# baowj-678/koordinator

Measured on AMD Instinct MI355X. Metric: pods placed/sec + (pod,node) Filter+Score evals/sec at 50k nodes, 1-8 GPUs, higher is better.
Workload: dtype int64; 1 GPU; config4: 50000 nodes x 100000 pods, 30% BE, NodeResourcesFit + LoadAwareScheduling, shipped scheduler-config.yaml profile; nodes=50000, pods=100000, batch_pods=24, pipeline_lag=2, parallelism=node-shard x1

## Files before the change

### koordinator_amd/csrc/api.hip

```cpp
#include <hip/hip_runtime.h>
#include <rccl/rccl.h>

#include <algorithm>
#include <array>
#include <cmath>
#include <condition_variable>
#include <memory>
#include <mutex>
#include <cstdio>
#include <cstdlib>
#include <cstring>
#include <chrono>
#include <string>
#include <unordered_map>
#include <vector>

#include "../../include/koordhip.h"
#include "cls.h"
#include "diag.h"
#include "diag_ext.h"
#include "reasons.h"
#include "preempt.h"
#include "kernels.h"
#include "place_plan.hpp"
// ... 2028 lines not shown
  int e = place_staged_impl(c);
  c->diag_valid = !e;
  if (e && c->group) c->group->abort();
  if (!e && std::getenv("KOORDHIP_PMC_REPLAY") && std::getenv("KOORDHIP_SERIAL")) e = pmc_replay(c);
  return e;
}

}

namespace {

kh::PlaceKnobs read_place_knobs() {
  const auto on = [](const char *name) { return std::getenv(name) != nullptr; };
  const auto num = [](const char *name, int32_t unset) {
    const char *v = std::getenv(name);
    return v ? std::atoi(v) : unset;
  };
  kh::PlaceKnobs k;
  k.SERIAL = on("KOORDHIP_SERIAL"), k.ROUND_LAUNCH = on("KOORDHIP_ROUND_LAUNCH");
  k.ONE_EVAL_STREAM = on("KOORDHIP_ONE_EVAL_STREAM"), k.CLS_OFF = on("KOORDHIP_CLS_OFF");
  k.SHARD_LOCAL_SIM = on("KOORDHIP_SHARD_LOCAL_SIM"), k.SHARD_FORCE = on("KOORDHIP_SHARD_FORCE");
  k.LAG1 = on("KOORDHIP_LAG1"), k.LAG2 = on("KOORDHIP_LAG2"), k.EXT_SEQ = on("KOORDHIP_EXT_SEQ");
  k.CHAIN_OFF = on("KOORDHIP_CHAIN_OFF"), k.STAMPS = on("KOORDHIP_STAMPS");
  k.NO_PRELOAD = on("KOORDHIP_NO_PRELOAD"), k.NO_KEY_TABLES = on("KOORDHIP_NO_KEY_TABLES");
  k.EXT_LEAD = num("KOORDHIP_EXT_LEAD", k.EXT_LEAD);
  k.CHAIN_PASSES = num("KOORDHIP_CHAIN_PASSES", k.CHAIN_PASSES);
  k.TRACE_POD = num("KOORDHIP_TRACE_POD", k.TRACE_POD);
  return k;
}

kh::PlaceFacts place_facts(const koordhip_ctx *c) {
  kh::PlaceFacts f;
  f.n = c->n, f.batch = c->batch, f.n_staged = c->n_staged, f.world = c->world, f.n_cu = c->n_cu;
  f.nbins = c->nbins, f.monotone = c->monotone;
  f.n_classes = (int32_t)c->cls_rep.size(), f.n_ext = (int32_t)c->ext_idx.size();
  f.has_comm = c->comm != nullptr, f.has_comm2 = c->comm2 != nullptr, f.has_group = c->group != nullptr;
  f.side = c->side, f.resv = c->resv, f.side_mode = kh::side_mode(c->dc);
  f.seq_profile = c->seq_profile, f.seq_ext_only = c->seq_ext_only, f.seq_snap = c->seq_snap;
  f.staged_ext = c->staged_ext, f.staged_ext_dev = c->staged_ext_dev, f.podx_staged = c->podx_staged;
  f.staged_reserve = c->staged_reserve, f.resv_dev_slot = c->d.dv.rslot != nullptr;
  f.resolve_lds_bytes = kh::resolve_lds_bytes;
  f.cls_run_lds = kh::cls_run_lds;
  return f;
}

int ensure_devout(koordhip_ctx *c) {
// ... 367 lines not shown
  HIP_TRY(hipMemsetAsync(pc->sync, 0, kh::kPipeSyncBytes, c->stream));
  HIP_TRY(hipEventRecord(c->ev_start, c->stream));
  HIP_TRY(hipStreamWaitEvent(c->rstream, c->ev_start, 0));
  if (plan.two) HIP_TRY(hipStreamWaitEvent(c->stream2, c->ev_start, 0));
  if (plan.rounds <= 0) return 0;
  if (plan.cls) {
    if (int e = cls_plan(c, plan.P, plan.lag, plan.K)) return e;
    if (int e = cls_alloc(c, c->n)) return e;
    if (int e = cls_reset(c)) return e;
    HIP_TRY(hipEventRecord(c->ev_start, c->stream));
    HIP_TRY(hipStreamWaitEvent(c->stream2, c->ev_start, 0));
    return 0;
  }
  for (int slot = 0; slot < (plan.two ? 2 : 1); slot++) {
    hipStream_t es = slot ? c->stream2 : c->stream;
    if (int e = eval_buffers(c, std::min(plan.P, c->n_staged), pc->lo, pc->hi, slot, es, plan.K)) return e;
    if (c->eval_fused) HIP_TRY(hipMemsetAsync(c->d_etk_sync[slot], 0, 2 * kh::kSelMaxPods * sizeof(uint32_t), es));
  }
  return 0;
}

int launch_resolve_rounds(koordhip_ctx *c, const PlaceCall &pc, int32_t r0, int32_t r1, int32_t mono, int32_t lag,
                          hipStream_t s) {
  HIP_TRY(kh::launch_resolve(c->dc, c->d, c->d_desc, c->d_pods, c->n_staged, pc.plan.P, pc.plan.K, r0, r1,
                             pc.plan.exch ? c->d_final : c->d_lists, (int64_t)kListBuf, mono, lag, pc.sync, c->d_mod,
                             c->d_out, c->d_cpus, c->d_dbg, pc.knobs.TRACE_POD, pc.knobs.NO_PRELOAD,
                             pc.knobs.NO_KEY_TABLES, s));
  c->resolve_kernel = kh::last_resolve_kernel();
  return 0;
}

int enqueue_resolve(koordhip_ctx *c, PlaceCall *pc) {
  if (!pc->plan.persistent || pc->plan.rounds <= 0) return 0;
  if (int e = timed_begin(c, TK_RESOLVE, c->rstream, &pc->res_tm)) return e;
  return launch_resolve_rounds(c, *pc, 0, pc->plan.rounds, pc->plan.mono, pc->plan.lag, c->rstream);
}

int enqueue_class_lists(koordhip_ctx *c, const PlaceCall &pc) {
  const kh::PlacePlan &plan = pc.plan;
  if (!plan.cls || plan.rounds <= 0) return 0;
  hipStream_t cs = c->stream;
  int32_t tm = -1;
  if (int e = timed_begin(c, TK_SCAN, cs, &tm)) return e;
  HIP_TRY(kh::launch_cls_run(c->dc, c->d, c->d_cls_pod, (int32_t)c->cls_rep.size(), c->d_plan + c->plan_off[0],
                             c->d_plan + c->plan_off[1], c->d_plan + c->plan_off[2], c->d_pod_cls, c->d_out, plan.lag,
                             plan.P, c->n_staged, c->d_cls_buf, c->d_cls_meta, plan.K, c->monotone, c->d_lists,
                             (int64_t)kListBuf, cls_sync(c, pc.sync), c->d_dbg ? c->d_dbg + 64 : nullptr, cs));
// ... 148 lines not shown
  if (plan.cls) {
    uint64_t q[32];
    HIP_TRY(hipMemcpy(q, c->d_dbg + 64, sizeof(q), hipMemcpyDeviceToHost));
    const double nl = (double)std::max<uint64_t>(q[7], 1), nc = (double)std::max<uint64_t>(q[15], 1);
    std::fprintf(stderr, "[koordhip stamps] class lists, cycles per launch (workgroup 0, %llu launches): buffer %.0f  log %.0f  "
                 "touched keys %.0f  compaction %.0f  sort %.0f  merge %.0f  outputs %.0f | builds (%llu): histogram %.0f  "
                 "fine %.0f  emit %.0f  sort %.0f  write %.0f\n", (unsigned long long)q[7], q[0] / nl, q[1] / nl, q[2] / nl,
                 q[3] / nl, q[4] / nl, q[5] / nl, q[6] / nl, (unsigned long long)q[15], q[8] / nc, q[9] / nc, q[10] / nc,
                 q[11] / nc, q[12] / nc);
  }
  {
    uint64_t q[4] = {0, 0, 0, 0}, rw[8] = {0, 0, 0, 0, 0, 0, 0, 0};
    HIP_TRY(hipMemcpy(q, c->d_dbg + 90, sizeof(q), hipMemcpyDeviceToHost));
    HIP_TRY(hipMemcpy(rw, c->d_dbg + 107, sizeof(rw), hipMemcpyDeviceToHost));
    std::fprintf(stderr, "[koordhip stamps] chain re-walks: walk + keys %llu (entries + claims %llu, row + evaluation "
                 "%llu)  winners' rows %llu cycles | winner rows loaded from HBM %llu\n", (unsigned long long)rw[0],
                 (unsigned long long)rw[5], (unsigned long long)rw[6], (unsigned long long)rw[1],
                 (unsigned long long)rw[2]);
    std::fprintf(stderr, "[koordhip stamps] chained decisions: %llu cycles, %llu pods resolved | claim tables %llu  "
                 "re-walks %llu  re-check + closure %llu  final table %llu | rounds with a lazy "
                 "claim table %llu\n", (unsigned long long)h[62],
                 (unsigned long long)h[63], (unsigned long long)q[0], (unsigned long long)q[1],
                 (unsigned long long)q[2], (unsigned long long)q[3], (unsigned long long)rw[7]);
  }
  if (plan.ext_pipe) {
    uint64_t q[8];
    HIP_TRY(hipMemcpy(q, c->d_dbg + 80, sizeof(q), hipMemcpyDeviceToHost));
    const double np = (double)std::max<uint64_t>(q[6], 1);
    std::fprintf(stderr, "[koordhip stamps] device pods (k_ext_pre / k_ext_final): %llu, resolve cycles from the "
                 "hand-off to the answer %llu (%.0f per pod) | final launch per pod: workgroup 0 evaluate + fold "
                 "%.0f | last workgroup: decide + publish %.0f  device commit %.0f\n",
                 (unsigned long long)h[31], (unsigned long long)h[30], h[31] ? (double)h[30] / h[31] : 0.0,
                 q[0] / np, q[3] / np, q[4] / np);
    uint64_t r[16];
    HIP_TRY(hipMemcpy(r, c->d_dbg + 96, sizeof(r), hipMemcpyDeviceToHost));
    std::fprintf(stderr, "[koordhip stamps] device-pod finals: workgroups with a full (device) re-evaluation %llu, "
                 "their re-evaluation %.2f us each\n", (unsigned long long)r[14], r[14] ? r[15] * 0.01 / r[14] : 0.0);
    const double nb = (double)std::max<uint64_t>(r[10], 1);
    std::fprintf(stderr, "[koordhip stamps] device-pod finals, us: request seen -> last workgroup arrived %.2f per pod | "
                 "per workgroup: -> gate seen %.2f  X marked %.2f  re-evaluated %.2f  folded + arrived %.2f\n",
                 r[5] * 0.01 / np, r[6] * 0.01 / nb, r[7] * 0.01 / nb, r[8] * 0.01 / nb, r[9] * 0.01 / nb);
    std::fprintf(stderr, "[koordhip stamps] device-pod hand-offs, us per pod: the request seen -> published %.2f | "
                 "requests already set when the final's first workgroup started: %llu of %llu | pre-evaluation "
                 "published after the request: %llu pods, waited %.2f us each\n",
                 r[2] * 0.01 / np, (unsigned long long)r[0], (unsigned long long)q[6], (unsigned long long)r[1],
                 r[1] ? r[3] * 0.01 / r[1] : 0.0);
// ... 979 lines not shown
```

### koordinator_amd/csrc/kernels.h

```cpp
#pragma once
#include <hip/hip_runtime.h>

#include "eval.hpp"
#include "place_plan.hpp"

namespace kh {

struct PrepIn {
  const int64_t *used_m[2];
  const int64_t *total_m[2];
  const int64_t *prod_used_m[2];
  const int64_t *thr[2];
  const int64_t *prod_thr[2];
  const uint8_t *la_flags;
};

hipError_t launch_prep_flags(const PrepIn &in, const DevNodes &d, const int32_t *rows, int32_t m, hipStream_t s);
hipError_t launch_eval_full(const DevCfg &c, const DevNodes &d, const DevPod *pods, int32_t n_pods,
                            uint8_t *status, int32_t *scores, hipStream_t s);
int32_t scan_chunks(int R, int32_t lo, int32_t hi);
hipError_t launch_scan(int R, const DevCfg &c, const DevNodes &d, const DevPod *pods, int32_t n_pods, int32_t lo,
                       int32_t hi, uint16_t *S, int64_t s_stride, uint16_t *Mx, int32_t m_stride, hipStream_t s);
struct PipeSync;
constexpr int kSelGMax = 16;
constexpr int kSelMaxPods = 64;
constexpr size_t kSelPartKeys = (size_t)kSelMaxPods * kSelGMax * 128;
int32_t select_split_groups(int32_t m, int32_t G);
hipError_t launch_select_split(const uint16_t *S, int64_t s_stride, int32_t lo, int32_t m, int32_t n_pods, int32_t k,
                               int32_t nbins, const uint16_t *Mx, int32_t m_stride, int32_t nchunks, int32_t G,
                               uint64_t *part, uint32_t *cnt, uint64_t *out, PipeSync *sync, int32_t sel_par,
                               hipStream_t s);
int32_t eval_topk_slices(int VT, int32_t lo, int32_t hi);
int eval_topk_vt(int nm, int32_t n_cu, int32_t n_pods, int32_t lo, int32_t hi, int32_t k, int knob);
hipError_t launch_eval_topk(const DevCfg &c, const DevNodes &d, const DevPod *pods, int32_t n_pods, int32_t lo,
                            int32_t hi, int32_t k, int VT, uint64_t *part, int32_t *pcnt, uint32_t *arrive,
                            uint64_t *out, PipeSync *sync, int32_t sel_par, int G, uint64_t *dbg, hipStream_t s);
hipError_t launch_topk_merge(const uint64_t *in, int64_t pod_stride, int64_t list_stride, int32_t n_pods, int32_t L,
                             int32_t k, int32_t score_bits, uint64_t *out, PipeSync *sync, int32_t sel_par,
                             hipStream_t s);
template <typename T>
hipError_t launch_scatter(T *dst, const T *src, const int32_t *idx, int32_t m, hipStream_t s);
hipError_t launch_scatter_rows(void *dst, const void *src, const int32_t *idx, int32_t m, int32_t bytes, hipStream_t s);
int side_mode(const DevCfg &c);
const char *last_eval_kernel();
const char *last_resolve_kernel();

int32_t resolve_lds_bytes(int32_t n_pods_max, int32_t k, int32_t n_nodes, int nm, int32_t lag);
hipError_t launch_resolve(const DevCfg &c, const DevNodes &d, const DevNodes *d_desc, const DevPod *pods, int32_t total, int32_t P, int32_t k,
                          int32_t r_begin, int32_t r_end, const uint64_t *lists0, int64_t list_buf, int32_t monotone,
                          int32_t lag, PipeSync *sync, int32_t *mbuf, int32_t *out_node, uint64_t *out_cpus, uint64_t *dbg,
                          int32_t trace, bool no_preload, bool no_key_tables, hipStream_t s);
hipError_t launch_wait_resolved(PipeSync *sync, int32_t rounds, hipStream_t s);
constexpr size_t kPipeSyncBytes = 384 + 4 * (1 + 128);
constexpr int kPipeSyncErrWord = 3;
constexpr int kPipeSyncExtReqWord = 32, kPipeSyncExtDoneWord = 64;
hipError_t launch_commit(const DevCfg &c, const DevNodes &d, const DevPod *pod, int32_t node, int32_t sign,
                         uint64_t *cpus, int32_t *rc, hipStream_t s);

}
```

### koordinator_amd/csrc/kernels.hip

```cpp
#include <hip/hip_runtime.h>

#include <algorithm>
#include <cstdio>

#include "eval.hpp"
#include "karg.hpp"
#include "kernels.h"
#include "pipe.hpp"
#include "rows.hpp"

namespace kh {


__device__ __forceinline__ uint64_t shfl_u64(uint64_t v, int src) {
  uint32_t lo = __shfl((uint32_t)v, src, 64);
  uint32_t hi = __shfl((uint32_t)(v >> 32), src, 64);
  return ((uint64_t)hi << 32) | lo;
}
__device__ __forceinline__ uint64_t shfl_up_u64(uint64_t v, int d) {
  uint32_t lo = __shfl_up((uint32_t)v, d, 64);
  uint32_t hi = __shfl_up((uint32_t)(v >> 32), d, 64);
  return ((uint64_t)hi << 32) | lo;
}
__device__ __forceinline__ uint64_t shfl_xor_u64(uint64_t v, int m) {
// ... 1135 lines not shown
static_assert(sizeof(NV) == RES_WORDS * 8, "NV row = 20 words");
static_assert(offsetof(NV, r) == 40 && offsetof(NV, nz_cpu) == 80 && offsetof(NV, la_u_cpu) == 112 &&
                  offsetof(NV, la_up_cpu) == 128 && offsetof(NV, a_pods) == 144 && offsetof(NV, npods) == 148 &&
                  offsetof(NV, flags) == 152,
              "NV word layout");

__device__ __forceinline__ NV slot_row(const NV &src) {
  NV v = src;
  uint32_t f = v.flags & ~(uint32_t)(NF_OVER_CPU | NF_OVER_MEM | NF_OVER_EPH);
  if (v.r[KOORDHIP_RES_CPU] > v.a[KOORDHIP_RES_CPU]) f |= NF_OVER_CPU;
  if (v.r[KOORDHIP_RES_MEM] > v.a[KOORDHIP_RES_MEM]) f |= NF_OVER_MEM;
  if (v.r[KOORDHIP_RES_EPH] > v.a[KOORDHIP_RES_EPH]) f |= NF_OVER_EPH;
  v.flags = f;
  return v;
}

struct ResLds {
  int32_t dep;
  int32_t lists, pods, prev_rows, prev_numa, cur_rows, cur_numa, hash_node, hash_slot, pre_rows, pre_numa, pre_node,
      dec_key, dec_n, dec_src, dec_e, dec_c, moved, mhash, gbits, kpre, ktab, ready, classes, modmap, total;
  int32_t kwide;
  int32_t overlap, lists2, pods2, pre_rows2, pre_numa2, pre_node2;
  int32_t ptab;
};

__host__ __device__ inline int32_t res_align(int32_t x) { return (x + 15) & ~15; }

__host__ __device__ inline int32_t res_ptab_bytes(int32_t nrow) {
  if (nrow == 0) return res_align((int32_t)offsetof(DevNodes, nu));
  return nrow == (int32_t)sizeof(NumaRow) ? res_align((int32_t)offsetof(DevNodes, rv)) : 0;
}

__host__ __device__ inline ResLds res_lds(int32_t n_pods_max, int32_t kp, int32_t n_nodes, int32_t nrow,
                                          bool overlap = false, bool tables = true, int32_t lag = 1,
                                          bool wide = false, bool chain = true) {
  const bool numa = nrow > 0;
  ResLds o;
  int32_t at = 0;
  const int32_t bitmap = res_align(((n_nodes + 31) >> 5) * 4);
  o.lists = at;
  at += res_align(n_pods_max * kp * 8);
  o.pods = at;
  at += res_align(n_pods_max * (int32_t)sizeof(DevPod));
  const int32_t rows_b = res_align(lag * n_pods_max * (int32_t)sizeof(NV));
  const int32_t numa_b = numa ? res_align(lag * n_pods_max * nrow) : 0;
  o.prev_rows = at;
// ... 4 lines not shown
  at += rows_b + numa_b;
  o.hash_node = at;
  at += RES_HASH * 4;
  o.hash_slot = at;
  at += RES_HASH * 4;
  o.pre_rows = at;
  at += res_align(RES_PRE * (int32_t)sizeof(NV));
  o.pre_numa = at;
  at += numa ? res_align(RES_PRE * nrow) : 0;
  o.pre_node = at;
  at += RES_PRE * 4;
  o.dec_key = at;
  at += RES_MAXP_ROUND * 8;
  o.dec_n = at;
  at += RES_MAXP_ROUND * 4;
  o.dec_src = at;
  at += RES_MAXP_ROUND * 4;
  o.dec_e = at;
  at += RES_MAXP_ROUND * RES_WE * 4;
  o.dec_c = at;
  at += RES_MAXP_ROUND * 4;
  o.dep = chain ? at : -1;
  at += chain ? RES_MAXP_ROUND * 8 : 0;
  o.moved = at;
  at += RES_MAXP_ROUND * 4;
  o.mhash = at;
  at += 2 * RES_MAXP_ROUND * 4;
  o.gbits = at;
  at += bitmap;
  o.kpre = o.ktab = -1;
  o.kwide = wide ? 1 : 0;
  o.ready = at;
  at += RES_MAXP_ROUND * 4;
  if (tables) {
    o.kpre = at;
    at += RES_MAXP_ROUND * RES_MAXP_ROUND * (wide ? 4 : 2);
    o.ktab = at;
    at += RES_MAXP_ROUND * RES_MAXP_ROUND * (wide ? 4 : 2);
  }
  o.classes = at;
  at += numa ? NUMA_LDS_CLASSES * (int32_t)sizeof(DevNumaClass) : 0;
  o.modmap = at;
  at += bitmap;
  o.ptab = res_ptab_bytes(nrow) ? at : -1;
  at += res_ptab_bytes(nrow);
  o.overlap = overlap ? 1 : 0;
  o.lists2 = o.pods2 = o.pre_rows2 = o.pre_numa2 = o.pre_node2 = 0;
  if (overlap) {
    o.lists2 = at;
    at += res_align(n_pods_max * kp * 8);
    o.pods2 = at;
    at += res_align(n_pods_max * (int32_t)sizeof(DevPod));
    o.pre_rows2 = at;
    at += res_align(RES_PRE * (int32_t)sizeof(NV));
    o.pre_numa2 = at;
    at += numa ? res_align(RES_PRE * nrow) : 0;
    o.pre_node2 = at;
    at += RES_PRE * 4;
  }
  o.total = at;
  return o;
}

__device__ __forceinline__ uint32_t res_hash(int32_t node) { return ((uint32_t)node * 2654435761u) >> 24; }
__device__ __forceinline__ DevPod uniform_pod(const DevPod &src) {
  DevPod p;
  const uint32_t *s = reinterpret_cast<const uint32_t *>(&src);
  uint32_t *o = reinterpret_cast<uint32_t *>(&p);
#pragma unroll
  for (int i = 0; i < (int)(sizeof(DevPod) / 4); i++) o[i] = __builtin_amdgcn_readfirstlane(s[i]);
  return p;
}
__device__ __forceinline__ bool xbit(const uint32_t *m, int32_t nd) { return (m[nd >> 5] >> (nd & 31)) & 1u; }
__device__ __forceinline__ uint64_t ktab_key(uint32_t v, int32_t nd) {
  return v ? ((uint64_t)v << 32) | (uint64_t)(0xFFFFFFFFu - (uint32_t)nd) : 0ull;
}

__global__ void k_wait_resolved(PipeSync *sy, int32_t rounds) {
  if (threadIdx.x == 0) (void)wait_at_least(&sy->res_round, rounds, sy);
}

template <int NM, bool DBG>
__global__ __launch_bounds__(res_threads<NM>()) void k_resolve(DevCfg c, const DevNodes *__restrict__ dn, int32_t n_nodes,
                                                                 const DevNumaClass *__restrict__ ncls, const DevPod *__restrict__ pods,
                                                                 int32_t total, int32_t P, int32_t k, int32_t kp,
                                                                 int32_t r_begin, int32_t r_end,
                                                                 int32_t *__restrict__ mbuf,
                                                                 const uint64_t *__restrict__ lists0,
                                                                 int64_t list_buf, int32_t monotone, int32_t lag,
                                                                 PipeSync *sy, ResLds ofs, int32_t *__restrict__ out_node,
                                                                 uint64_t *__restrict__ out_cpus,
                                                                 uint64_t *__restrict__ dbg, int32_t trace) {
  constexpr int RES_THREADS = res_threads<NM>();
  constexpr bool NUMA = NM != 0, ZONES = NM == 2;
  if constexpr (!DBG) dbg = nullptr;
  using NR = side_row_t<NM>;
  (void)trace;
  extern __shared__ __attribute__((aligned(16))) char lds[];
  uint64_t *lk = reinterpret_cast<uint64_t *>(lds + ofs.lists);
  DevPod *lpod = reinterpret_cast<DevPod *>(lds + ofs.pods);
  NV *prow = reinterpret_cast<NV *>(lds + ofs.prev_rows);
  NR *pnr = reinterpret_cast<NR *>(lds + ofs.prev_numa);
  NV *mrow = reinterpret_cast<NV *>(lds + ofs.cur_rows);
  NR *mnr = reinterpret_cast<NR *>(lds + ofs.cur_numa);
  int32_t *hnode = reinterpret_cast<int32_t *>(lds + ofs.hash_node);
  int32_t *hslot = reinterpret_cast<int32_t *>(lds + ofs.hash_slot);
  NV *pre = reinterpret_cast<NV *>(lds + ofs.pre_rows);
// ... 32 lines not shown
  __shared__ int32_t seg_w[RES_MAXP_ROUND];
  __shared__ int32_t ckey[RES_HASH], cval[RES_HASH];
  __shared__ int32_t sh_mp, sh_stop, sh_done, sh_chain;
  __shared__ uint64_t sh_rsv;
  const int t = threadIdx.x, lane = lane_id();
  const int32_t words = (n_nodes + 31) >> 5;
  const int32_t HP = max(1, RES_PRE / P);
  auto nodes = [&]() -> decltype(auto) {
    if constexpr (NM <= 2) {
      return *reinterpret_cast<const DevNodes *>(lds + ofs.ptab);
    } else {
      const DevNodes *p = dn;
      asm volatile("" : "+s"(p));
      return DevNodes(*p);
    }
  };
  if constexpr (NM <= 2) {
    constexpr int PW = (int)((NUMA ? offsetof(DevNodes, rv) : offsetof(DevNodes, nu)) / 8);
    static_assert(PW <= RES_THREADS, "one 8-byte word of the pointer table per thread");
    if (t < PW) reinterpret_cast<uint64_t *>(lds + ofs.ptab)[t] = reinterpret_cast<const uint64_t *>(dn)[t];
  }
  const bool two = kp > 64;
  const bool chain_on = (monotone & 2) && ofs.dep >= 0;
  const uint64_t t_kernel = (dbg && t == 0) ? stamp() : 0;
  if (t == 0) {
    sh_mp = r_begin > 0 ? min(mbuf[0], P) : 0;
    sh_stop = 0;
  }
  for (int32_t x = t; x < words; x += RES_THREADS) {
    modmap[x] = 0;
    gbits[x] = 0;
  }
  for (int32_t x = t; x < RES_MAXP_ROUND; x += RES_THREADS) {
    moved[x] = 0;
    ready[x] = 0;
  }
  for (int32_t x = t; x < RES_HASH; x += RES_THREADS) {
    ckey[x] = -1;
    cval[x] = 64;
  }
  const DevNumaClass *cls = ncls;
  if constexpr (NUMA) {
    const int32_t nc = dn->nu.ncls;
    if (nc <= NUMA_LDS_CLASSES) {
      uint4 *dst = reinterpret_cast<uint4 *>(lds + ofs.classes);
      const uint4 *src = reinterpret_cast<const uint4 *>(ncls);
// ... 20 lines not shown
  auto word_doff = [](int q) -> int32_t {
    if (q >= 5 && q < 10) return (q - 5) * 8;
    if (q == 10 || q == 11) return (int32_t)offsetof(DevPod, nz_cpu_m) + (q - 10) * 8;
    if (q == 14 || q == 16) return (int32_t)offsetof(DevPod, est_cpu);
    if (q == 15 || q == 17) return (int32_t)offsetof(DevPod, est_mem);
    return -1;
  };
  const int32_t doff = word_doff(lane);
  uint64_t c_pro = 0, c_wait = 0, c_loop = 0, c_rel = 0, c_hash = 0, c_wb = 0;
  uint64_t c_w1wait = 0, c_w1load = 0, c_bar = 0;
  uint64_t c_l[4] = {0, 0, 0, 0};
  uint64_t n_slow = 0, n_miss = 0, n_staged = 0, n_bulk = 0, n_tab = 0;
  uint64_t c_g[2] = {0, 0};
  uint64_t c_nx[8] = {0, 0, 0, 0, 0, 0, 0, 0};
  uint64_t c_p[3] = {0, 0, 0}, n_p2 = 0, n_conf = 0, n_slowc = 0, n_void = 0;
  uint64_t c_cand = 0, n_evpass = 0, n_tready = 0;
  uint64_t c_gc[3] = {0, 0, 0}, n_ghit = 0;
  uint64_t c_chain = 0;
  uint64_t c_ch[4] = {0, 0, 0, 0};
  uint64_t c_rw[4] = {0, 0, 0, 0}, n_chbm = 0;
  uint64_t n_lazy = 0;
  uint64_t c_ext = 0, n_ext = 0;
  auto load_round = [&](int32_t rr, int32_t rp0, int32_t rn, uint64_t *Lk, DevPod *Lp, NV *Pr, NR *Pn,
                        int32_t *Pnode, int32_t tid, int32_t nth) {
    const uint64_t *L = lists0 + (size_t)(rr & (2 * lag - 1)) * list_buf;
    const int32_t tot = rn * k;
    uint64_t he[2] = {0, 0};
    bool hv[2];
#pragma unroll
    for (int u = 0; u < 2; u++) {
      const int32_t sl = tid + u * nth, j = sl / HP, q = sl - j * HP;
      hv[u] = sl < RES_PRE && j < rn && q < k;
      if (u * nth < RES_PRE) he[u] = L[min(j * k + q, tot - 1)];
    }
    constexpr int LB = 6;
    const uint4 *L4 = reinterpret_cast<const uint4 *>(L);
    const int32_t n16 = (tot + 1) >> 1;
    auto put = [&](int32_t e, uint64_t v) {
      if (e < tot) {
        const int32_t j = e / k, q = e - j * k;
        Lk[j * kp + q] = v;
      }
    };
    auto put2 = [&](int32_t x, const uint4 &w) {
      if (x < n16) {
        put(2 * x, ((uint64_t)w.y << 32) | w.x);
        put(2 * x + 1, ((uint64_t)w.w << 32) | w.z);
      }
    };
// ... 63 lines not shown
        }
      }
      Pnode[sl] = nd[u];
    }
    for (int32_t sl = tid + 2 * nth; sl < RES_PRE; sl += nth) {
      const int32_t j = sl / HP, q = sl - j * HP;
      int32_t n1 = -1;
      if (j < rn && q < k) {
        const uint64_t e = L[(size_t)j * k + q];
        if (e != 0) n1 = key_node(e);
      }
      if (n1 >= 0) {
        NV v1;
        load_row(v1, nodes(), n1);
        Pr[sl] = v1;
        if constexpr (NUMA) {
          NR rr2;
          load_side_row<NM>(rr2, nodes(), n1);
          Pn[sl] = rr2;
        }
      }
      Pnode[sl] = n1;
    }
  };
  auto prev_slot = [&](int32_t nd) -> int32_t {
    uint32_t h = res_hash(nd);
    for (;;) {
      const int32_t x = hnode[h];
      if (x == nd) return hslot[h];
      if (x < 0) return -1;
      h = (h + 1) & (RES_HASH - 1);
    }
  };
  for (int32_t r = r_begin, p0 = r_begin * P; r < r_end && p0 < total; r++, p0 += P) {
    const int32_t n_pods = min(P, total - p0);
    const bool preloaded = ofs.overlap && r > r_begin;
    const uint64_t t_w0 = (dbg && t == 0) ? stamp() : 0;
    if (!preloaded) {
      if (t == 0 && !wait_at_least(&sy->sel[r & 1], P * (r >> 1) + n_pods, sy)) sh_stop = 1;
      __syncthreads();
    }
    if (sh_stop) return;
    const uint64_t t_entry = (dbg && t == 0) ? stamp() : 0;
    const int32_t mp = sh_mp;
    if (!preloaded) load_round(r, p0, n_pods, lk, lpod, pre, prenr, pre_node, t, RES_THREADS);
    for (int32_t x = t; x < RES_HASH; x += RES_THREADS) hnode[x] = -1;
    if (t == 0) {
      sh_done = 0;
      sh_chain = 0;
    }
    __syncthreads();
    if (t < mp) {
      const int32_t nd = pnode[t];
      uint32_t h = res_hash(nd);
      while (atomicCAS(&hnode[h], -1, nd) != -1) h = (h + 1) & (RES_HASH - 1);
      hslot[h] = t;
    }
    __syncthreads();
    const uint64_t t_a = (dbg && t == 0) ? stamp() : 0;
    if (mp > 0 && t < RES_PRE) {
      const int32_t nd = pre_node[t];
      if (nd >= 0 && prev_slot(nd) >= 0) pre_node[t] = -1;
    }
    for (int32_t base = 0; base < n_pods * RES_WE; base += RES_THREADS) {
      const int32_t x = base + t;
      const int32_t l = x / RES_WE, q = x - l * RES_WE;
      const bool live = l < n_pods;
      const uint64_t e = (live && q < kp) ? lk[l * kp + q] : 0ull;
      const int32_t nd = e ? key_node(e) : -1;
      const bool inx = e != 0 && xbit(modmap, nd);
      const int g = lane & ~(RES_WE - 1);
      const uint32_t bx = (uint32_t)(__ballot(live && e != 0 && !inx) >> g) & 0xFFu;
      const uint32_t bz = (uint32_t)(__ballot(live && e == 0) >> g) & 0xFFu;
      const int f = bx ? __builtin_ctz(bx) : RES_WE, z = bz ? __builtin_ctz(bz) : RES_WE;
      const bool general = f == RES_WE && z == RES_WE;
      const bool walked = live && !general && (q < min(f, z) || (q == f && f < z));
      uint64_t key = 0;
      int32_t ms = -1;
      if (walked) {
        if (q < min(f, z)) {
          ms = prev_slot(nd);
          const DevPod pod = lpod[l];
          key = make_key(eval_row<NM>(pod, slot_row(prow[ms]), pnr[ms], cls, c), nd);
        } else {
          key = e;
        }
      }
      uint64_t mx = key;
#pragma unroll
      for (int m = 1; m < RES_WE; m <<= 1) {
        const uint64_t o = shfl_xor_u64(mx, m);
        mx = o > mx ? o : mx;
      }
      if (live) {
        dec_e[l * RES_WE + q] = walked ? nd : -1;
        if (walked && key == mx && mx != 0) {
          int32_t src;
          if (ms >= 0) {
            src = -ms - 1;
          } else if (q < HP && pre_node[l * HP + q] == nd) {
            src = l * HP + q;
          } else {
            src = l * HP;
            if (dbg) n_p2++;
            NV v;
            load_row(v, nodes(), nd);
            pre[src] = v;
            if constexpr (NUMA) {
              NR nr;
              load_side_row<NM>(nr, nodes(), nd);
              prenr[src] = nr;
            }
            pre_node[src] = nd;
          }
          dec_src[l] = src;
        }
        if (q == 0) {
          const int32_t dn = general ? -1 : (f < z ? f + 1 : z);
          dec_key[l] = mx;
          dec_n[l] = dn;
          if (mx == 0 || dn < 0) dec_src[l] = 0;
          const uint32_t fl = lpod[l].flags;
          bool slow = !monotone || dn < 0;
          if constexpr (NM == 0) slow = slow || (fl & KH_POD_EXT) != 0u;
          if constexpr (NUMA) {
            slow = slow || (numa_on(c) && ((fl & KOORDHIP_POD_CPUSET) || c.zones) &&
                            !(fl & (KOORDHIP_POD_NUMA_SKIP | KOORDHIP_POD_NUMA_ERROR)));
          }
          if constexpr (NM >= 3) {
            slow = slow || lpod[l].resv_match != 0ull;
          }
          dec_c[l] = slow ? 2 : 0;
          if (!slow && mx != 0) {
            const int32_t sw = key_node(mx);
            uint32_t h = res_hash(sw);
            for (;;) {
              const int32_t prev = atomicCAS(&ckey[h], -1, sw);
              if (prev == -1 || prev == sw) {
                atomicMin(&cval[h], l);
                break;
              }
              h = (h + 1) & (RES_HASH - 1);
            }
          }
        }
      }
    }
    const uint64_t t_p1 = (dbg && t == 0) ? stamp() : 0;
    __syncthreads();
    const uint64_t t_p2 = (dbg && t == 0) ? stamp() : 0;
    for (int32_t x = t; x < n_pods * RES_WE; x += RES_THREADS) {
      const int32_t l = x / RES_WE;
      const int32_t y = dec_e[x];
      if (y >= 0 && !(dec_c[l] & 2)) {
        uint32_t h = res_hash(y);
        for (;;) {
          const int32_t xk = ckey[h];
          if (xk == y) {
            if (cval[h] < l) atomicOr(&dec_c[l], 1);
            break;
          }
          if (xk < 0) break;
          h = (h + 1) & (RES_HASH - 1);
        }
      }
    }
    __syncthreads();
    uint64_t *dep = ofs.dep >= 0 ? reinterpret_cast<uint64_t *>(lds + ofs.dep) : nullptr;
    if (dep)
      for (int32_t x = t; x < n_pods; x += RES_THREADS) dep[x] = 0ull;
    if (dbg && t == 0) {
      const uint64_t t_p3 = stamp();
      c_hash += t_a - t_entry;
      c_pro += t_p3 - t_a;
      c_wait += t_entry - t_w0;
      c_p[0] += t_p1 - t_a;
      c_p[1] += t_p2 - t_p1;
      c_p[2] += t_p3 - t_p2;
    }
    if (t < 64) {
      __builtin_amdgcn_s_setprio(3);
      auto wsync = [&]() {
        asm volatile("s_waitcnt lgkmcnt(0)" ::: "memory");
        __builtin_amdgcn_fence(__ATOMIC_SEQ_CST, "wavefront");
      };
      bool claims_stale = false;
      auto claims = [&]() {
        for (int32_t x = lane; x < RES_HASH; x += 64) {
          ckey[x] = -1;
          cval[x] = 64;
        }
        wsync();
        if (lane < n_pods && dec_c[lane] == 0 && dec_key[lane] != 0ull) {
          const int32_t sw2 = key_node(dec_key[lane]);
          uint32_t h = res_hash(sw2);
          for (;;) {
            const int32_t prev = atomicCAS(&ckey[h], -1, sw2);
            if (prev == -1 || prev == sw2) {
              atomicMin(&cval[h], lane);
              break;
            }
            h = (h + 1) & (RES_HASH - 1);
          }
        }
        wsync();
      };
      if (chain_on) {
        const uint64_t t_c0 = dbg ? stamp() : 0;
        auto claimer_of = [&](int32_t y) -> int32_t {
          uint32_t q = res_hash(y);
          for (;;) {
            const int32_t xk = ckey[q];
            if (xk == y) return cval[q];
            if (xk == -1) return 64;
            q = (q + 1) & (RES_HASH - 1);
          }
        };
        auto drop_conflicting = [&]() {
          if (lane < n_pods && dec_c[lane] == 1 && dec_key[lane] != 0ull) {
            const int32_t y = key_node(dec_key[lane]);
            uint32_t q = res_hash(y);
            for (;;) {
              const int32_t xk = ckey[q];
              if (xk == y) {
                if (cval[q] == lane) ckey[q] = -2;
                break;
              }
              if (xk == -1) break;
              q = (q + 1) & (RES_HASH - 1);
            }
          }
// ... 622 lines not shown
        pgen[sidx] = r - 1;
      }
      moved[lane] = 0;
      const uint64_t t_rel = dbg ? stamp() : 0;
      if (dbg) c_wb += t_rel - t_wb;
      if (lane == 0) {
        sh_mp = nm + ns;
        asm volatile("s_waitcnt vmcnt(0)" ::: "memory");
        __hip_atomic_store(&sy->res_round, r + 1, __ATOMIC_RELAXED, __HIP_MEMORY_SCOPE_AGENT);
      }
      if (dbg) {
        const uint64_t t_end = stamp();
        c_rel += t_end - t_rel;
        c_loop += t_end - t_loop;
      }
    } else if (t < 64 * (1 + res_loaders<NM>())) {
      if (ofs.overlap && r + 1 < r_end && p0 + P < total) {
        const int32_t np2 = min(P, total - (p0 + P));
        int ok = 1;
        const uint64_t t1 = dbg ? stamp() : 0;
        if (lane == 0) ok = wait_at_least(&sy->sel[(r + 1) & 1], P * ((r + 1) >> 1) + np2, sy) ? 1 : 0;
        const uint64_t t2 = dbg ? stamp() : 0;
        if (__builtin_amdgcn_readfirstlane(ok)) {
          load_round(r + 1, p0 + P, np2, lk2, lpod2, pre2, prenr2, pre_node2, t - 64, 64 * res_loaders<NM>());
          if (dbg) {
            asm volatile("s_waitcnt vmcnt(0) lgkmcnt(0)" ::: "memory");
            c_w1load += stamp() - t2;
          }
        } else if (lane == 0) {
          sh_stop = 1;
        }
        if (dbg) c_w1wait += t2 - t1;
      }
    } else {
      const int hw = __builtin_amdgcn_readfirstlane((t >> 6) - 1 - res_loaders<NM>()),
                nh = RES_THREADS / 64 - 1 - res_loaders<NM>();
      if (chain_on)
        while (!__hip_atomic_load(&sh_chain, __ATOMIC_ACQUIRE, __HIP_MEMORY_SCOPE_WORKGROUP)) __builtin_amdgcn_s_sleep(1);
      uint64_t todo = __ballot(lane < n_pods && dec_c[lane] == 1);
      for (int32_t x = 0; x < hw && todo; x++) todo &= todo - 1ull;
      for (; have_tables && todo;) {
        const int32_t l = (int32_t)__builtin_ctzll(todo);
        for (int32_t x = 0; x < nh && todo; x++) todo &= todo - 1ull;
        if (__hip_atomic_load(&sh_done, __ATOMIC_RELAXED, __HIP_MEMORY_SCOPE_WORKGROUP)) break;
        const DevPod pod = uniform_pod(lpod[l]);
        for (int32_t b0 = 0; b0 < l + mp; b0 += 64) {
          const int32_t x = b0 + lane;
// ... 21 lines not shown
        if (lane == 0) __hip_atomic_store(&ready[l], 1, __ATOMIC_RELEASE, __HIP_MEMORY_SCOPE_WORKGROUP);
      }
    }
    const uint64_t t_bar = (dbg && t == 0) ? stamp() : 0;
    __syncthreads();
    if (dbg && t == 0) c_bar += stamp() - t_bar;
    for (int32_t x = t; x < RES_MAXP_ROUND; x += RES_THREADS) ready[x] = 0;
    if (ofs.overlap) {
      uint64_t *a = lk;
      lk = lk2;
      lk2 = a;
      DevPod *b = lpod;
      lpod = lpod2;
      lpod2 = b;
      NV *c2 = pre;
      pre = pre2;
      pre2 = c2;
      NR *d2 = prenr;
      prenr = prenr2;
      prenr2 = d2;
      int32_t *e2 = pre_node;
      pre_node = pre_node2;
      pre_node2 = e2;
    }
    {
      NV *x = prow;
      prow = mrow;
      mrow = x;
      NR *y = pnr;
      pnr = mnr;
      mnr = y;
    }
  }
  if (t <= RES_MAXP_ROUND && t <= sh_mp) mbuf[t] = t == 0 ? sh_mp : pnode[t - 1];
  if (dbg && n_p2) atomicAdd((unsigned long long *)&dbg[51], (unsigned long long)n_p2);
  if (dbg && n_evpass) atomicAdd((unsigned long long *)&dbg[57], (unsigned long long)n_evpass);
  if (dbg && t == 64) {
    atomicAdd((unsigned long long *)&dbg[27], (unsigned long long)c_w1wait);
    atomicAdd((unsigned long long *)&dbg[28], (unsigned long long)c_w1load);
  }
  if (dbg && t == 0) {
    atomicAdd((unsigned long long *)&dbg[0], (unsigned long long)c_pro);
    atomicAdd((unsigned long long *)&dbg[1], (unsigned long long)c_wait);
    atomicAdd((unsigned long long *)&dbg[2], (unsigned long long)c_hash);
    atomicAdd((unsigned long long *)&dbg[4], (unsigned long long)c_loop);
    atomicAdd((unsigned long long *)&dbg[5], (unsigned long long)n_slow);
// ... 324 lines not shown
  }
  hipLaunchKernelGGL(k_topk_merge, dim3(n_pods), dim3(MERGE_THREADS), lds, s, in, pod_stride, list_stride, L, k,
                     score_bits, out, sync, sel_par);
  return hipGetLastError();
}

static inline int32_t list_stride(int32_t k) { return (k + 7) & ~7; }

int side_mode(const DevCfg &c) {
  if (c.resv) return c.resv_cpus ? 5 : (c.resv_slots > 1 ? 4 : 3);
  if (!((c.filt | c.score) & KOORDHIP_PLUGIN_NUMA)) return 0;
  return c.zones ? 2 : 1;
}

static int32_t side_row_bytes(int nm) {
  return nm >= 4 ? (int32_t)sizeof(NumaRowR4) : nm == 3 ? (int32_t)sizeof(NumaRowR) : (nm ? (int32_t)sizeof(NumaRow) : 0);
}

int32_t resolve_lds_bytes(int32_t n_pods_max, int32_t k, int32_t n_nodes, int nm, int32_t lag) {
  const int32_t kp = list_stride(k);
  return res_lds(n_pods_max, kp, n_nodes, side_row_bytes(nm), false, false, lag, false, nm <= 2).total;
}

hipError_t launch_resolve(const DevCfg &c, const DevNodes &d, const DevNodes *d_desc, const DevPod *pods, int32_t total, int32_t P, int32_t k,
                          int32_t r_begin, int32_t r_end, const uint64_t *lists0, int64_t list_buf, int32_t monotone,
                          int32_t lag, PipeSync *sync, int32_t *mbuf, int32_t *out_node, uint64_t *out_cpus, uint64_t *dbg,
                          int32_t trace, bool no_preload, bool no_key_tables, hipStream_t s) {
  if (total <= 0 || r_end <= r_begin) return hipSuccess;
  if (P > RES_MAXP_ROUND || P < 1 || k > RES_MAXP || k < 1) return hipErrorInvalidValue;
  if (lag < 1 || lag > 2 || lag * P > RES_MAXP_ROUND || (lag > 1 && (k < 3 * P || r_begin != 0)))
    return hipErrorInvalidValue;
  const int32_t kp = list_stride(k);
  const int nm = side_mode(c);
  const int32_t nrow = side_row_bytes(nm);
  const bool pre = r_end - r_begin > 1 && !no_preload;
  const bool tab = !no_key_tables;
  const bool wide = c.wide_keys != 0;
  const bool chain = nm <= 2;
  ResLds o = res_lds(P, kp, d.n, nrow, pre, tab, lag, wide, chain);
  if (o.total > RES_LDS_MAX) o = res_lds(P, kp, d.n, nrow, false, tab, lag, wide, chain);
  if (o.total > RES_LDS_MAX) o = res_lds(P, kp, d.n, nrow, pre, false, lag, wide, chain);
  if (o.total > RES_LDS_MAX) o = res_lds(P, kp, d.n, nrow, false, false, lag, wide, chain);
  static bool attr[12] = {};
  const int ai = nm * 2 + (dbg ? 1 : 0);
  if (!attr[ai]) {
    const void *f = dbg ? (nm == 5   ? (const void *)k_resolve<5, true>
                           : nm == 4 ? (const void *)k_resolve<4, true>
                           : nm == 3 ? (const void *)k_resolve<3, true>
                           : nm == 2 ? (const void *)k_resolve<2, true>
                                     : (nm == 1 ? (const void *)k_resolve<1, true> : (const void *)k_resolve<0, true>))
                        : (nm == 5   ? (const void *)k_resolve<5, false>
                           : nm == 4 ? (const void *)k_resolve<4, false>
                           : nm == 3 ? (const void *)k_resolve<3, false>
                           : nm == 2 ? (const void *)k_resolve<2, false>
                                     : (nm == 1 ? (const void *)k_resolve<1, false> : (const void *)k_resolve<0, false>));
    const hipError_t e = hipFuncSetAttribute(f, hipFuncAttributeMaxDynamicSharedMemorySize, RES_LDS_MAX);
    if (e != hipSuccess) return e;
    attr[ai] = true;
  }
  if (o.total > RES_LDS_MAX) return hipErrorInvalidValue;
#define KH_RESOLVE_D(NN, DD)                                                                                  \
  do {                                                                                                        \
    note_kernel(g_resolve_name, DD ? "kh::k_resolve<%d, true>" : "kh::k_resolve<%d, false>", NN);                \
    hipLaunchKernelGGL((k_resolve<NN, DD>), dim3(1), dim3(res_threads<NN>()), o.total, s, c, d_desc, d.n, d.nu.cls, \
                       pods, total, P, k, kp, r_begin, r_end, mbuf, lists0, list_buf, monotone, lag, sync, o, out_node, \
                       out_cpus, dbg, trace);                                                                   \
  } while (0)
#define KH_RESOLVE(NN)       \
  if (dbg)                   \
    KH_RESOLVE_D(NN, true);  \
  else                       \
    KH_RESOLVE_D(NN, false)
  if (nm == 5)
    KH_RESOLVE(5);
  else if (nm == 4)
    KH_RESOLVE(4);
  else if (nm == 3)
    KH_RESOLVE(3);
  else if (nm == 2)
    KH_RESOLVE(2);
  else if (nm == 1)
    KH_RESOLVE(1);
  else
    KH_RESOLVE(0);
#undef KH_RESOLVE
#undef KH_RESOLVE_D
  return hipGetLastError();
}
// ... 14 lines not shown
```

### koordinator_amd/csrc/place_plan.hpp

```cpp
#pragma once

#include <algorithm>
#include <cstddef>
#include <cstdint>

namespace kh {

constexpr int32_t kMaxBatch = 64;
constexpr int32_t kResolveMaxK = 128;
constexpr int32_t kClsTarget = 2048;
constexpr int32_t kClsLead = 12;
constexpr int32_t kResolveLdsBudget = 157 * 1024;
constexpr size_t kClsLdsBudget = 150 * 1024;

constexpr int32_t cls_amax(int32_t P, int32_t K) { return (kClsTarget - K) / P; }

struct PlaceKnobs {
  bool SERIAL = false, ROUND_LAUNCH = false, ONE_EVAL_STREAM = false, CLS_OFF = false;
  bool SHARD_LOCAL_SIM = false, SHARD_FORCE = false, LAG1 = false, LAG2 = false;
  bool EXT_SEQ = false, CHAIN_OFF = false, STAMPS = false;
  bool NO_PRELOAD = false, NO_KEY_TABLES = false;
  int32_t EXT_LEAD = 0;
  int32_t CHAIN_PASSES = 1;
  int32_t TRACE_POD = -1;
};

struct PlaceFacts {
  int32_t n = 0, batch = 1, n_staged = 0, world = 1, n_cu = 256, nbins = 2, monotone = 1;
  int32_t n_classes = 0;
  int32_t n_ext = 0;
  bool has_comm = false, has_comm2 = false, has_group = false;
  bool side = false, resv = false;
  int side_mode = 0;
  bool seq_profile = false, seq_ext_only = false, seq_snap = false;
  bool staged_ext = false, staged_ext_dev = false, podx_staged = false, staged_reserve = false;
  bool resv_dev_slot = false;
  int32_t (*resolve_lds_bytes)(int32_t, int32_t, int32_t, int, int32_t) = nullptr;
  size_t (*cls_run_lds)(int32_t, int32_t) = nullptr;
};

struct PlacePlan {
  bool seq = false;
  bool ext_pipe = false;
// ... 33 lines not shown
  p->rounds = (f.n_staged + P - 1) / P;
}

inline int32_t ext_lead(const PlaceKnobs &k, int32_t lag) { return std::max(lag, k.EXT_LEAD); }

inline PlacePlan plan_place(const PlaceFacts &f, const PlaceKnobs &k) {
  PlacePlan p;
  p.ext_pipe = ext_pipe_eligible(f, k);
  p.seq = f.staged_reserve || f.seq_snap || (f.seq_profile && (!f.seq_ext_only || f.staged_ext) && !p.ext_pipe);
  if (p.seq) {
    p.lag = 0, p.P = 1, p.K = 1, p.rounds = f.n_staged, p.lead = 0;
    return p;
  }
  p.serial = k.SERIAL;
  p.persistent = !p.serial && !f.has_group && !k.ROUND_LAUNCH;
  const bool cls_fit = cls_eligible(f, k);
  const bool local_sim = f.world == 1 && !f.has_comm && k.SHARD_LOCAL_SIM;
  p.local = (f.world > 1 || local_sim) && !f.has_group && p.persistent && cls_fit && !k.SHARD_FORCE;
  p.exch = (f.world > 1 || f.has_comm) && !p.local;
  p.two = p.persistent && (!p.exch || f.has_comm2) && !k.ONE_EVAL_STREAM;
  round_shape(f, k, &p);
  p.cls = p.two && !p.exch && cls_fit && cls_amax(p.P, p.K) >= 4 * kClsLead + 2;
  p.lead = ext_lead(k, p.lag);
  p.mono = f.monotone | ((f.monotone && !k.CHAIN_OFF) ? 2 : 0) | (f.monotone ? ((k.CHAIN_PASSES & 3) << 2) : 0);
  p.tstride = std::max<int32_t>(1, (p.rounds + 255) / 256);
  if (f.resolve_lds_bytes(p.P, p.K, f.n, f.side_mode, p.lag) > kResolveLdsBudget) {
    p.err = 1;
    p.msg = "snapshot too large for the resolve kernel's LDS";
  }
  return p;
}

}
```

Baseline: 1.753 million pods/s.

## Speculate same-class pod conflicts in resolve by assuming predecessors claim earlier candidates

Adds same-class speculation to the resolve kernel. Each pod gets a rank word in LDS listing earlier same-class pods in its round. A pod of rank r assumes those predecessors claim its first r candidates, so it evaluates its list from the (r+1)th candidate using the preloaded row plus its own delta. Guesses are checked against the actual claimers and cascaded through a dependency mask, and wrong ones fall back to the existing slow path. This is meant to cut the chained re-walks and extra decision passes when many pods in a batch share a class, at the cost of more LDS, extra ballots and per-round rank computation.

```diff
diff --git a/koordinator_amd/csrc/api.hip b/koordinator_amd/csrc/api.hip
--- a/koordinator_amd/csrc/api.hip
+++ b/koordinator_amd/csrc/api.hip
@@ -2074,6 +2074,7 @@
   k.SHARD_LOCAL_SIM = on("KOORDHIP_SHARD_LOCAL_SIM"), k.SHARD_FORCE = on("KOORDHIP_SHARD_FORCE");
   k.LAG1 = on("KOORDHIP_LAG1"), k.LAG2 = on("KOORDHIP_LAG2"), k.EXT_SEQ = on("KOORDHIP_EXT_SEQ");
   k.CHAIN_OFF = on("KOORDHIP_CHAIN_OFF"), k.STAMPS = on("KOORDHIP_STAMPS");
+  k.SAMECLS_OFF = on("KOORDHIP_SAMECLS_OFF");
   k.NO_PRELOAD = on("KOORDHIP_NO_PRELOAD"), k.NO_KEY_TABLES = on("KOORDHIP_NO_KEY_TABLES");
   k.EXT_LEAD = num("KOORDHIP_EXT_LEAD", k.EXT_LEAD);
   k.CHAIN_PASSES = num("KOORDHIP_CHAIN_PASSES", k.CHAIN_PASSES);
@@ -2487,7 +2488,8 @@
 
 int launch_resolve_rounds(koordhip_ctx *c, const PlaceCall &pc, int32_t r0, int32_t r1, int32_t mono, int32_t lag,
                           hipStream_t s) {
-  HIP_TRY(kh::launch_resolve(c->dc, c->d, c->d_desc, c->d_pods, c->n_staged, pc.plan.P, pc.plan.K, r0, r1,
+  const int32_t *pod_cls = c->cls_rep.empty() ? nullptr : c->d_pod_cls;
+  HIP_TRY(kh::launch_resolve(c->dc, c->d, c->d_desc, c->d_pods, pod_cls, c->n_staged, pc.plan.P, pc.plan.K, r0, r1,
                              pc.plan.exch ? c->d_final : c->d_lists, (int64_t)kListBuf, mono, lag, pc.sync, c->d_mod,
                              c->d_out, c->d_cpus, c->d_dbg, pc.knobs.TRACE_POD, pc.knobs.NO_PRELOAD,
                              pc.knobs.NO_KEY_TABLES, s));
@@ -2682,6 +2684,13 @@
                  "claim table %llu\n", (unsigned long long)h[62],
                  (unsigned long long)h[63], (unsigned long long)q[0], (unsigned long long)q[1],
                  (unsigned long long)q[2], (unsigned long long)q[3], (unsigned long long)rw[7]);
+    uint64_t sp[7] = {0, 0, 0, 0, 0, 0, 0};
+    HIP_TRY(hipMemcpy(sp, c->d_dbg + 116, sizeof(sp), hipMemcpyDeviceToHost));
+    std::fprintf(stderr, "[koordhip stamps] same-class speculation: made %llu  validated %llu  invalidated %llu | "
+                 "given up: no head row %llu  walk past the entries %llu  winner assumed-claimed %llu  winner row in "
+                 "HBM %llu\n", (unsigned long long)sp[0], (unsigned long long)sp[1], (unsigned long long)sp[2],
+                 (unsigned long long)sp[3], (unsigned long long)sp[4], (unsigned long long)sp[5],
+                 (unsigned long long)sp[6]);
   }
   if (plan.ext_pipe) {
     uint64_t q[8];
diff --git a/koordinator_amd/csrc/kernels.h b/koordinator_amd/csrc/kernels.h
--- a/koordinator_amd/csrc/kernels.h
+++ b/koordinator_amd/csrc/kernels.h
@@ -46,7 +46,8 @@
 const char *last_resolve_kernel();
 
 int32_t resolve_lds_bytes(int32_t n_pods_max, int32_t k, int32_t n_nodes, int nm, int32_t lag);
-hipError_t launch_resolve(const DevCfg &c, const DevNodes &d, const DevNodes *d_desc, const DevPod *pods, int32_t total, int32_t P, int32_t k,
+hipError_t launch_resolve(const DevCfg &c, const DevNodes &d, const DevNodes *d_desc, const DevPod *pods, const int32_t *pod_cls,
+                          int32_t total, int32_t P, int32_t k,
                           int32_t r_begin, int32_t r_end, const uint64_t *lists0, int64_t list_buf, int32_t monotone,
                           int32_t lag, PipeSync *sync, int32_t *mbuf, int32_t *out_node, uint64_t *out_cpus, uint64_t *dbg,
                           int32_t trace, bool no_preload, bool no_key_tables, hipStream_t s);
diff --git a/koordinator_amd/csrc/kernels.hip b/koordinator_amd/csrc/kernels.hip
--- a/koordinator_amd/csrc/kernels.hip
+++ b/koordinator_amd/csrc/kernels.hip
@@ -1181,6 +1181,7 @@
   int32_t kwide;
   int32_t overlap, lists2, pods2, pre_rows2, pre_numa2, pre_node2;
   int32_t ptab;
+  int32_t rank, rank2;
 };
 
 __host__ __device__ inline int32_t res_align(int32_t x) { return (x + 15) & ~15; }
@@ -1231,6 +1232,9 @@
   at += RES_MAXP_ROUND * 4;
   o.dep = chain ? at : -1;
   at += chain ? RES_MAXP_ROUND * 8 : 0;
+  o.rank = chain ? at : -1;
+  at += chain ? RES_MAXP_ROUND * 8 : 0;
+  o.rank2 = o.rank;
   o.moved = at;
   at += RES_MAXP_ROUND * 4;
   o.mhash = at;
@@ -1266,6 +1270,10 @@
     at += numa ? res_align(RES_PRE * nrow) : 0;
     o.pre_node2 = at;
     at += RES_PRE * 4;
+    if (chain) {
+      o.rank2 = at;
+      at += RES_MAXP_ROUND * 8;
+    }
   }
   o.total = at;
   return o;
@@ -1292,6 +1300,7 @@
 template <int NM, bool DBG>
 __global__ __launch_bounds__(res_threads<NM>()) void k_resolve(DevCfg c, const DevNodes *__restrict__ dn, int32_t n_nodes,
                                                                  const DevNumaClass *__restrict__ ncls, const DevPod *__restrict__ pods,
+                                                                 const int32_t *__restrict__ pod_cls,
                                                                  int32_t total, int32_t P, int32_t k, int32_t kp,
                                                                  int32_t r_begin, int32_t r_end,
                                                                  int32_t *__restrict__ mbuf,
@@ -1370,6 +1379,10 @@
   }
   const bool two = kp > 64;
   const bool chain_on = (monotone & 2) && ofs.dep >= 0;
+  static_assert(RES_WE == 8, "a pod's rank word: one rank byte + RES_WE - 1 predecessor bytes");
+  const bool spec_on = NM == 0 && chain_on && ofs.rank >= 0 && pod_cls != nullptr && !(monotone & 16);
+  uint64_t *rk = reinterpret_cast<uint64_t *>(lds + (ofs.rank >= 0 ? ofs.rank : 0));
+  uint64_t *rk2 = reinterpret_cast<uint64_t *>(lds + (ofs.rank2 >= 0 ? ofs.rank2 : 0));
   const uint64_t t_kernel = (dbg && t == 0) ? stamp() : 0;
   if (t == 0) {
     sh_mp = r_begin > 0 ? min(mbuf[0], P) : 0;
@@ -1436,9 +1449,12 @@
   uint64_t n_lazy = 0;
   uint64_t c_ext = 0, n_ext = 0;
   auto load_round = [&](int32_t rr, int32_t rp0, int32_t rn, uint64_t *Lk, DevPod *Lp, NV *Pr, NR *Pn,
-                        int32_t *Pnode, int32_t tid, int32_t nth) {
+                        int32_t *Pnode, uint64_t *Rk, int32_t tid, int32_t nth) {
     const uint64_t *L = lists0 + (size_t)(rr & (2 * lag - 1)) * list_buf;
     const int32_t tot = rn * k;
+    const int32_t rl = t - 64;
+    int32_t mycls = -1;
+    if (Rk && rl >= 0 && rl < rn) mycls = pod_cls[rp0 + rl];
     uint64_t he[2] = {0, 0};
     bool hv[2];
 #pragma unroll
@@ -1548,6 +1564,18 @@
       }
       Pnode[sl] = n1;
     }
+    if (Rk && rl >= 0 && rl < 64) {
+      uint64_t w = 0;
+      int32_t cnt = 0;
+      for (int32_t j = 0; j < rn; j++) {
+        const int32_t cj = __builtin_amdgcn_readlane(mycls, j);
+        if (j < rl && cj == mycls) {
+          if (cnt < RES_WE - 1) w |= (uint64_t)j << (8 * (cnt + 1));
+          cnt++;
+        }
+      }
+      if (rl < rn) Rk[rl] = w | (uint64_t)cnt;
+    }
   };
   auto prev_slot = [&](int32_t nd) -> int32_t {
     uint32_t h = res_hash(nd);
@@ -1569,7 +1597,12 @@
     if (sh_stop) return;
     const uint64_t t_entry = (dbg && t == 0) ? stamp() : 0;
     const int32_t mp = sh_mp;
-    if (!preloaded) load_round(r, p0, n_pods, lk, lpod, pre, prenr, pre_node, t, RES_THREADS);
+    if (!preloaded) {
+      const bool first = r == r_begin;
+      load_round(r, p0, n_pods, lk, lpod, pre, prenr, pre_node, (spec_on && !first) ? rk : nullptr, t, RES_THREADS);
+      if (spec_on && first)
+        for (int32_t x = t; x < n_pods; x += RES_THREADS) rk[x] = 0ull;
+    }
     for (int32_t x = t; x < RES_HASH; x += RES_THREADS) hnode[x] = -1;
     if (t == 0) {
       sh_done = 0;
@@ -1600,14 +1633,49 @@
       const uint32_t bz = (uint32_t)(__ballot(live && e == 0) >> g) & 0xFFu;
       const int f = bx ? __builtin_ctz(bx) : RES_WE, z = bz ? __builtin_ctz(bz) : RES_WE;
       const bool general = f == RES_WE && z == RES_WE;
-      const bool walked = live && !general && (q < min(f, z) || (q == f && f < z));
+      bool spec = false;
+      int fw = f, gu = -1;
+      uint64_t rkw = 0;
+      if constexpr (NM == 0) {
+        if (spec_on) {
+          rkw = live ? rk[l] : 0ull;
+          const int rank = (int)(rkw & 0xFFull);
+          if (rank > 0 && !(lpod[l].flags & KH_POD_EXT)) {
+            uint32_t b = bx;
+            for (int u = 0; u < rank && b; u++) b &= b - 1u;
+            if (rank < RES_WE && b && __builtin_ctz(b) < z) {
+              spec = true;
+              fw = __builtin_ctz(b);
+            } else {
+              gu = 1;
+            }
+          }
+          if (__ballot(spec)) {
+            const bool nohead = spec && q < fw && !inx && !(q < HP && pre_node[l * HP + q] == nd);
+            if (spec && ((uint32_t)(__ballot(nohead) >> g) & 0xFFu)) {
+              spec = false;
+              fw = f;
+              gu = 0;
+            }
+          }
+        }
+      }
+      bool walked = live && !general && (q < min(fw, z) || (q == fw && fw < z));
+      bool assumed = spec && q < fw && !inx;
       uint64_t key = 0;
       int32_t ms = -1;
       if (walked) {
-        if (q < min(f, z)) {
-          ms = prev_slot(nd);
+        if (q < min(fw, z)) {
           const DevPod pod = lpod[l];
-          key = make_key(eval_row<NM>(pod, slot_row(prow[ms]), pnr[ms], cls, c), nd);
+          NV v;
+          if (assumed) {
+            v = pre[l * HP + q];
+            apply_delta(v, pod, +1);
+          } else {
+            ms = prev_slot(nd);
+            v = slot_row(prow[ms]);
+          }
+          key = make_key(eval_row<NM>(pod, v, pnr[ms >= 0 ? ms : 0], cls, c), nd);
         } else {
           key = e;
         }
@@ -1617,6 +1685,31 @@
       for (int m = 1; m < RES_WE; m <<= 1) {
         const uint64_t o = shfl_xor_u64(mx, m);
         mx = o > mx ? o : mx;
+      }
+      if constexpr (NM == 0) {
+        if (__ballot(spec)) {
+          const bool win = spec && walked && key == mx && mx != 0;
+          const uint32_t brep = (uint32_t)(__ballot(win && assumed) >> g) & 0xFFu;
+          const uint32_t bhbm =
+              (uint32_t)(__ballot(win && q == fw && !(q < HP && pre_node[l * HP + q] == nd)) >> g) & 0xFFu;
+          const bool back = spec && (brep | bhbm) != 0u;
+          if (back) {
+            spec = false;
+            gu = brep ? 2 : 3;
+            fw = f;
+            assumed = false;
+            walked = q < min(f, z) || (q == f && f < z);
+            key = walked ? (q == f ? e : key) : 0ull;
+          }
+          if (__ballot(back)) {
+            mx = key;
+#pragma unroll
+            for (int m = 1; m < RES_WE; m <<= 1) {
+              const uint64_t o = shfl_xor_u64(mx, m);
+              mx = o > mx ? o : mx;
+            }
+          }
+        }
       }
       if (live) {
         dec_e[l * RES_WE + q] = walked ? nd : -1;
@@ -1642,9 +1735,22 @@
           dec_src[l] = src;
         }
         if (q == 0) {
-          const int32_t dn = general ? -1 : (f < z ? f + 1 : z);
+          const int32_t dn = general ? -1 : (fw < z ? fw + 1 : z);
           dec_key[l] = mx;
           dec_n[l] = dn;
+          if (ofs.dep >= 0) {
+            uint64_t dm = 0;
+            if (spec)
+              for (int u = 1; u <= (int)(rkw & 0xFFull); u++) dm |= 1ull << ((rkw >> (8 * u)) & 0xFFull);
+            reinterpret_cast<uint64_t *>(lds + ofs.dep)[l] = dm;
+          }
+          if constexpr (NM == 0) {
+            if (spec_on) rk[l] = (rkw & ~0xFFull) | (spec ? (uint64_t)(bx & ((1u << fw) - 1u)) : 0ull);
+            if (dbg) {
+              if (spec) atomicAdd((unsigned long long *)&dbg[116], 1ull);
+              if (gu >= 0) atomicAdd((unsigned long long *)&dbg[119 + gu], 1ull);
+            }
+          }
           if (mx == 0 || dn < 0) dec_src[l] = 0;
           const uint32_t fl = lpod[l].flags;
           bool slow = !monotone || dn < 0;
@@ -1679,22 +1785,31 @@
       const int32_t l = x / RES_WE;
       const int32_t y = dec_e[x];
       if (y >= 0 && !(dec_c[l] & 2)) {
+        int32_t cv = 64;
         uint32_t h = res_hash(y);
         for (;;) {
           const int32_t xk = ckey[h];
           if (xk == y) {
-            if (cval[h] < l) atomicOr(&dec_c[l], 1);
+            cv = cval[h];
             break;
           }
           if (xk < 0) break;
           h = (h + 1) & (RES_HASH - 1);
         }
+        bool bad = cv < l;
+        if constexpr (NM == 0) {
+          if (spec_on) {
+            const uint64_t w = rk[l];
+            const uint32_t am = (uint32_t)(w & 0xFFull);
+            const int32_t q = x - l * RES_WE;
+            if ((am >> q) & 1u) bad = cv != (int32_t)((w >> (8 * (1 + __popc(am & ((1u << q) - 1u))))) & 0xFFull);
+          }
+        }
+        if (bad) atomicOr(&dec_c[l], 1);
       }
     }
     __syncthreads();
     uint64_t *dep = ofs.dep >= 0 ? reinterpret_cast<uint64_t *>(lds + ofs.dep) : nullptr;
-    if (dep)
-      for (int32_t x = t; x < n_pods; x += RES_THREADS) dep[x] = 0ull;
     if (dbg && t == 0) {
       const uint64_t t_p3 = stamp();
       c_hash += t_a - t_entry;
@@ -1733,6 +1848,27 @@
       };
       if (chain_on) {
         const uint64_t t_c0 = dbg ? stamp() : 0;
+        if constexpr (NM == 0) {
+          if (spec_on) {
+            const bool lv = lane < n_pods;
+            const uint64_t dl = lv ? dep[lane] : 0ull;
+            const uint64_t made = __ballot(dl != 0ull);
+            if (made) {
+              uint64_t valid = __ballot(lv && dec_c[lane] == 0);
+              for (;;) {
+                const uint64_t bad = __ballot(((valid >> lane) & 1ull) && (dl & ~valid) != 0ull);
+                if (!bad) break;
+                valid &= ~bad;
+                if ((bad >> lane) & 1ull) dec_c[lane] = 1;
+              }
+              wsync();
+              if (dbg && lane == 0) {
+                atomicAdd((unsigned long long *)&dbg[117], (unsigned long long)__popcll(made & valid));
+                atomicAdd((unsigned long long *)&dbg[118], (unsigned long long)__popcll(made & ~valid));
+              }
+            }
+          }
+        }
         auto claimer_of = [&](int32_t y) -> int32_t {
           uint32_t q = res_hash(y);
           for (;;) {
@@ -2401,7 +2537,8 @@
         if (lane == 0) ok = wait_at_least(&sy->sel[(r + 1) & 1], P * ((r + 1) >> 1) + np2, sy) ? 1 : 0;
         const uint64_t t2 = dbg ? stamp() : 0;
         if (__builtin_amdgcn_readfirstlane(ok)) {
-          load_round(r + 1, p0 + P, np2, lk2, lpod2, pre2, prenr2, pre_node2, t - 64, 64 * res_loaders<NM>());
+          load_round(r + 1, p0 + P, np2, lk2, lpod2, pre2, prenr2, pre_node2, spec_on ? rk2 : nullptr, t - 64,
+                     64 * res_loaders<NM>());
           if (dbg) {
             asm volatile("s_waitcnt vmcnt(0) lgkmcnt(0)" ::: "memory");
             c_w1load += stamp() - t2;
@@ -2469,6 +2606,9 @@
       int32_t *e2 = pre_node;
       pre_node = pre_node2;
       pre_node2 = e2;
+      uint64_t *f2 = rk;
+      rk = rk2;
+      rk2 = f2;
     }
     {
       NV *x = prow;
@@ -2839,7 +2979,8 @@
   return res_lds(n_pods_max, kp, n_nodes, side_row_bytes(nm), false, false, lag, false, nm <= 2).total;
 }
 
-hipError_t launch_resolve(const DevCfg &c, const DevNodes &d, const DevNodes *d_desc, const DevPod *pods, int32_t total, int32_t P, int32_t k,
+hipError_t launch_resolve(const DevCfg &c, const DevNodes &d, const DevNodes *d_desc, const DevPod *pods, const int32_t *pod_cls,
+                          int32_t total, int32_t P, int32_t k,
                           int32_t r_begin, int32_t r_end, const uint64_t *lists0, int64_t list_buf, int32_t monotone,
                           int32_t lag, PipeSync *sync, int32_t *mbuf, int32_t *out_node, uint64_t *out_cpus, uint64_t *dbg,
                           int32_t trace, bool no_preload, bool no_key_tables, hipStream_t s) {
@@ -2880,7 +3021,7 @@
   do {                                                                                                        \
     note_kernel(g_resolve_name, DD ? "kh::k_resolve<%d, true>" : "kh::k_resolve<%d, false>", NN);                \
     hipLaunchKernelGGL((k_resolve<NN, DD>), dim3(1), dim3(res_threads<NN>()), o.total, s, c, d_desc, d.n, d.nu.cls, \
-                       pods, total, P, k, kp, r_begin, r_end, mbuf, lists0, list_buf, monotone, lag, sync, o, out_node, \
+                       pods, pod_cls, total, P, k, kp, r_begin, r_end, mbuf, lists0, list_buf, monotone, lag, sync, o, out_node, \
                        out_cpus, dbg, trace);                                                                   \
   } while (0)
 #define KH_RESOLVE(NN)       \
diff --git a/koordinator_amd/csrc/place_plan.hpp b/koordinator_amd/csrc/place_plan.hpp
--- a/koordinator_amd/csrc/place_plan.hpp
+++ b/koordinator_amd/csrc/place_plan.hpp
@@ -19,6 +19,7 @@
   bool SERIAL = false, ROUND_LAUNCH = false, ONE_EVAL_STREAM = false, CLS_OFF = false;
   bool SHARD_LOCAL_SIM = false, SHARD_FORCE = false, LAG1 = false, LAG2 = false;
   bool EXT_SEQ = false, CHAIN_OFF = false, STAMPS = false;
+  bool SAMECLS_OFF = false;
   bool NO_PRELOAD = false, NO_KEY_TABLES = false;
   int32_t EXT_LEAD = 0;
   int32_t CHAIN_PASSES = 1;
@@ -98,7 +99,8 @@
   round_shape(f, k, &p);
   p.cls = p.two && !p.exch && cls_fit && cls_amax(p.P, p.K) >= 4 * kClsLead + 2;
   p.lead = ext_lead(k, p.lag);
-  p.mono = f.monotone | ((f.monotone && !k.CHAIN_OFF) ? 2 : 0) | (f.monotone ? ((k.CHAIN_PASSES & 3) << 2) : 0);
+  p.mono = f.monotone | ((f.monotone && !k.CHAIN_OFF) ? 2 : 0) | (f.monotone ? ((k.CHAIN_PASSES & 3) << 2) : 0) |
+           ((f.monotone && k.SAMECLS_OFF) ? 16 : 0);
   p.tstride = std::max<int32_t>(1, (p.rounds + 255) / 256);
   if (f.resolve_lds_bytes(p.P, p.K, f.n, f.side_mode, p.lag) > kResolveLdsBudget) {
     p.err = 1;
```

After: 1.855 million pods/s (median of 6 runs). +5.8%, better.
